# DavidSlayback/po-brax

Hardware: AMD Instinct MI355X
Metric: env-steps/sec AntHeavenHell batch 65536 @1/2/4/8 GPU; % HBM roofline (higher is better)
Workload: dtype f32; 1 GPU; ant_heavenhell B=65536/GPU (global 65536), create(batch_size=B) autoreset chain, episode_length 1000, PBD 10 substeps, random uniform(-1,1) actions (threefry); env=ant_heavenhell, global_batch=65536, batch_per_gpu=65536, episode_length=1000, qp_storage=f32, parallelism=env-shard x1 (strong: global batch split), dynamics=pbd, obs_mask=none, obs_mask_columns=0, launch=hipGraph replay of the K steps

## Files before the change

__graft_entry__.py:

```python
from __future__ import annotations

import os
import subprocess
import sys
import sysconfig

ROOT = os.path.dirname(os.path.abspath(__file__))
PKG_ROOT = os.path.join(ROOT, "po-brax_amd")
CSRC = os.path.join(PKG_ROOT, "csrc")
LIB = os.path.join(PKG_ROOT, "po_brax_amd", "libpob.so")
HIP_SOURCES = ["pob_kernels.hip", "pob_system.cpp"]
HIP_DEPS = HIP_SOURCES + ["pob_math.h", "pob_mesh.h", "pob_physics.h", "pob_quad.h", "pob_octet.h", "pob_hexa.h", "pob_sys.h"]
HIPCC_FLAGS = ["--offload-arch=gfx950", "-O3", "-std=c++17", "-ffp-contract=off", "-fno-fast-math",
               "-fno-slp-vectorize", "-fPIC", "-shared", "-mcode-object-version=5", "-Wall",
               "-Wno-unused-result"]

if PKG_ROOT not in sys.path:
    sys.path.insert(0, PKG_ROOT)


def _stale(target, deps):
    if not os.path.exists(target):
        return True
    t = os.path.getmtime(target)
    return any(os.path.getmtime(d) > t for d in deps)


def build_lib(force: bool = False) -> str:
    deps = [os.path.join(CSRC, f) for f in HIP_DEPS] + [os.path.join(ROOT, "include", "pob.h")]
    if force or _stale(LIB, deps):
        hipcc = os.environ.get("HIPCC", "/opt/rocm/bin/hipcc")
        cmd = [hipcc, *HIPCC_FLAGS, "-o", LIB, *[os.path.join(CSRC, f) for f in HIP_SOURCES]]
        subprocess.check_call(cmd)
    return LIB

# ... 61 lines not shown
```

po-brax_amd/csrc/pob_kernels.hip:

```cpp
#include <hip/hip_fp16.h>
#include <hip/hip_runtime.h>

#include <climits>
#include <cstdio>
#include <cstdlib>
#include <cstring>
#include <mutex>
#include <new>
#include <type_traits>
#include <vector>

#include "../../include/pob.h"

#ifndef POB_QUAD_PRIO
#define POB_QUAD_PRIO 1
#endif
#ifndef POB_OCT_PRIO
#define POB_OCT_PRIO 1
#endif
#ifndef POB_HEX_PRIO
#define POB_HEX_PRIO 1
#endif
#include "pob_quad.h"
#include "pob_octet.h"
#include "pob_hexa.h"
#include "pob_physics.h"

namespace pob {
void default_params(pob_params &p);
const char *build_system(int kind, const pob_params &p, pob_sys &s);
int gather_grid(const pob_params &p, float *xyz, int cap);
}

struct pob_env {
  pob_sys sys;
  pob_sys *d_sys = nullptr;
  pob_params params;
  float *d_grid = nullptr;
  uint32_t *d_scratch = nullptr;
  int device = 0;
  int n_cu = 256;
};

#define POB_MIXED (-1)
#define POB_F_STAGED (1u << 16)
#define POB_F_INT_FORCE_FIXUP (1u << 30)
#define POB_F_INTERNAL (POB_F_STAGED | POB_F_INT_FORCE_FIXUP)
#define POB_F_PUBLIC (POB_F_EPISODE | POB_F_AUTORESET | POB_F_ZERO_STEPS_ON_DONE)

#define POB_STATE_FIELDS(X)                                                                    \
  X(pos) X(rot) X(vel) X(ang) X(obs) X(reward) X(done) X(steps) X(truncation) X(m0) X(m1) X(m2) \
  X(rng) X(first_pos) X(first_rot) X(first_vel) X(first_ang) X(first_obs) X(any_done) X(done_u8) X(trunc_i32) \
  X(m0_i32) X(m1_i32) X(any_done_clear) X(obs_masked) X(ovf_mark)

struct StatePtrs {
  float *pos, *rot, *vel, *ang, *obs, *reward, *done, *steps, *truncation, *m0, *m1, *m2;
  uint32_t *rng;
  float *first_pos, *first_rot, *first_vel, *first_ang, *first_obs;
  uint32_t *any_done;
  uint8_t *done_u8;
  int32_t *trunc_i32, *m0_i32, *m1_i32;
  uint32_t *any_done_clear;
  float *obs_masked;
  uint8_t *ovf_mark;
};
POB_D void store_obs_masked(csys_t &S, float *dst, const float *stg, const int rows, const int D, const int lane) {
  const int K = S.obs_mask_n;
  for (int r = 0; r < rows; ++r)
    for (int c = lane; c < K; c += 64) dst[(size_t)r * K + c] = stg[r * D + S.obs_mask[c]];
}
// ... 555 lines not shown
#pragma unroll
      for (int l = 0; l < QNB; ++l) {
        if (l == 0 && k != 0) continue;
        const int g = qbody_global(l, k);
        float *o = stg + (le * POB_NDYN + g) * c;
        if (reset_rows) {
          const float *F = arr == 0 ? in.first_pos : (arr == 1 ? in.first_rot : (arr == 2 ? in.first_vel : in.first_ang));
          const size_t src = (arr == 1 ? r4 : r3) + (size_t)g * c;
          for (int q = 0; q < c; ++q) o[q] = Q<QT>::ld(F, src + q);
        } else if (arr == 0) { o[0] = bd.x[l].x; o[1] = bd.x[l].y; o[2] = bd.x[l].z; }
        else if (arr == 1) { o[0] = bd.q[l].w; o[1] = bd.q[l].x; o[2] = bd.q[l].y; o[3] = bd.q[l].z; }
        else if (arr == 2) { o[0] = bd.v[l].x; o[1] = bd.v[l].y; o[2] = bd.v[l].z; }
        else { o[0] = bd.w[l].x; o[1] = bd.w[l].y; o[2] = bd.w[l].z; }
      }
    }
    wave_lds_sync();
    if (arr == 1) stage_store_dyn<QT, 4>(out.rot, (size_t)b_first * N * 4, N, nenv, stg, lane);
    else stage_store_dyn<QT, 3>(arr == 0 ? out.pos : (arr == 2 ? out.vel : out.ang), (size_t)b_first * N * 3, N,
                                nenv, stg, lane);
    wave_lds_sync();
  }
}

template <int KIND, typename QT, bool LEG = false, int MODE = 0>
POB_D void step_quad_body(csys_t *Sp, const int B, const StatePtrs &in, const float *__restrict__ act,
                          const StatePtrs &out, const uint32_t flags, const int L, const int gt, float *lds,
                          const float *legtab) {
  csys_t &S = *Sp;
  const int lane = (int)threadIdx.x & 63;
  POB_TS_DECL();
  POB_TS(0);
  float *stg = lds + ((int)threadIdx.x >> 6) * POB_STAGE_FLOATS;
  const QLds Ls{stg, lane};
  int b = gt >> 2;
  int k = gt & 3;
  const float *LT = legtab + k * POB_LEG_FLOATS;
  const float *WT = legtab + 4 * POB_LEG_FLOATS;
  const int kind = KIND != POB_MIXED ? KIND : S.kind;
  const int N = n_bodies<KIND>(S), D = obs_dim<KIND>(S);
  const int sh = obs_shift(kind);
  bool act_lane = b < B;
  int b_first = (gt - lane) >> 2;
  if (b_first >= B) return;
  if (MODE == 2 && out.ovf_mark[b_first] == 0) return;
  if (MODE == 1 && lane == 0) out.ovf_mark[b_first] = 0;
  int nenv = B - b_first < 16 ? B - b_first : 16;
  int le = b - b_first;
  int bl = act_lane ? b : B - 1, lel = bl - b_first;
  size_t r3 = (size_t)bl * N * 3, r4 = (size_t)bl * N * 4;
  auto rederive = [&]() {
    int g2 = gt;
    asm volatile("" : "+v"(g2));
    b = g2 >> 2;
    k = g2 & 3;
    act_lane = b < B;
    b_first = (g2 - (g2 & 63)) >> 2;
    nenv = B - b_first < 16 ? B - b_first : 16;
    le = b - b_first;
    bl = act_lane ? b : B - 1;
    lel = bl - b_first;
    r3 = (size_t)bl * N * 3;
    r4 = (size_t)bl * N * 4;
  };

  QBody bd;
  constexpr int NMAX = KIND == POB_HEAVENHELL ? 14 : (KIND == POB_TAG ? 12 : (KIND == POB_ANT ? 10 : POB_MAXB));
  constexpr int MAXI = (16 * NMAX * 4 + 255) / 256;
  if ((flags & POB_F_STAGED) && NMAX <= 16 && N == NMAX && 16 * N * 7 <= POB_STAGE_FLOATS) {
// ... 110 lines not shown
    };
    for (;;) {
    if (pass == 0) {
      bool near = false;
#pragma nounroll
      for (int it = 0; it < 2 * iters; ++it) {
#if POB_QUAD_PRIO == 1
        const int lvl = (it * 4) / (2 * iters);
        if (lvl == 0) __builtin_amdgcn_s_setprio(3);
        else if (lvl == 1) __builtin_amdgcn_s_setprio(2);
        else if (lvl == 2) __builtin_amdgcn_s_setprio(1);
        else __builtin_amdgcn_s_setprio(0);
#endif
        qpbd_substep<false, true>(Sp, LT, WT, bd, a, Ls, (it & 1) != 0, fric, &near);
      }
      if (!__any(near)) break;
      pass = 1;
      reload();
      continue;
    }
#ifndef POB_QUAD_SLOW_OOL
#define POB_QUAD_SLOW_OOL 1
#endif
    if (MODE == 1 && WALLS) {
      bool ovf = false;
#pragma nounroll
      for (int it = 0; it < 2 * iters; ++it) {
#if POB_QUAD_PRIO == 1
        const int lvl = (it * 4) / (2 * iters);
        if (lvl == 0) __builtin_amdgcn_s_setprio(3);
        else if (lvl == 1) __builtin_amdgcn_s_setprio(2);
        else if (lvl == 2) __builtin_amdgcn_s_setprio(1);
        else __builtin_amdgcn_s_setprio(0);
#endif
        qpbd_substep<WALLS, false, false>(Sp, LT, WT, bd, a, Ls, (it & 1) != 0, fric, nullptr, &ovf);
        if (__any(ovf)) break;
      }
      if (__any(ovf) || (flags & POB_F_INT_FORCE_FIXUP)) {
        if (lane == 0) out.ovf_mark[b_first] = 1;
        return;
      }
      break;
    }
    if (pass == 1 && WALLS && FASTP && MODE == 0) {
      bool ovf = false;
#pragma nounroll
// ... 188 lines not shown
    if (out.truncation) out.truncation[b] = t.trunc;
    if (out.m0) out.m0[b] = t.m0;
    if (out.m1) out.m1[b] = t.m1;
    if (out.m2) out.m2[b] = t.m2;
    out.rng[2 * b] = t.rng0;
    out.rng[2 * b + 1] = t.rng1;
    write_typed(out, b, t);
  }
  if (out.any_done) {
    const unsigned long long m = __ballot(act_lane && k == 0 && done != 0.0f);
    if (m != 0ull && lane == 0) atomicOr(out.any_done, 1u);
  }
  POB_TS_WRITE();
}

POB_D bool quad_block_marked(const int B, const uint8_t *mark, const int bt0) {
  bool any = false;
  for (int w = 0; w < (int)blockDim.x / 64; ++w) {
    const int bf = (bt0 + 64 * w) >> 2;
    if (bf < B) any = any | (mark[bf] != 0);
  }
  return any;
}
template <int KIND, typename QT, int MODE = 0>
__global__ __launch_bounds__(256, POB_QUAD_MIN_WAVES) void k_step_quad(const void *sysp, const int B,
                                                                       const StatePtrs in,
                                                                       const float *__restrict__ act,
                                                                       const StatePtrs out, const uint32_t flags,
                                                                       const int L) {
  __shared__ float lds[QL_FLOATS * 256];
  __shared__ __attribute__((aligned(16))) float legtab[POB_TAB_FLOATS];
  if (MODE == 2 && !quad_block_marked(B, out.ovf_mark, (int)(blockIdx.x * blockDim.x)))
    return;
  stage_leg_table((csys_t *)(size_t)sysp, legtab);
  step_quad_body<KIND, QT, false, MODE>((csys_t *)(size_t)sysp, B, in, act, out, flags, L,
                                        (int)(blockIdx.x * blockDim.x + threadIdx.x), lds, legtab);
}

template <typename QT>
__global__ __launch_bounds__(256, 3) void k_step_quad_ga3(const void *sysp, const int B, const StatePtrs in,
                                                          const float *__restrict__ act, const StatePtrs out,
                                                          const uint32_t flags, const int L) {
  __shared__ float lds[QL_FLOATS * 256];
  __shared__ __attribute__((aligned(16))) float legtab[POB_TAB_FLOATS];
  stage_leg_table((csys_t *)(size_t)sysp, legtab);
  step_quad_body<POB_GATHER, QT>((csys_t *)(size_t)sysp, B, in, act, out, flags, L,
                                 (int)(blockIdx.x * blockDim.x + threadIdx.x), lds, legtab);
}

template <int KIND, typename QT>
__global__ __launch_bounds__(256) void k_step_legacy(const void *sysp, const int B, const StatePtrs in,
                                                     const float *__restrict__ act, const StatePtrs out,
                                                     const uint32_t flags, const int L) {
  __shared__ float lds[QL_FLOATS * 256];
  __shared__ __attribute__((aligned(16))) float legtab[POB_TAB_FLOATS];
  stage_leg_table((csys_t *)(size_t)sysp, legtab);
  step_quad_body<KIND, QT, true>((csys_t *)(size_t)sysp, B, in, act, out, flags, L,
                                 (int)(blockIdx.x * blockDim.x + threadIdx.x), lds, legtab);
// ... 1420 lines not shown
    default: hipLaunchKernelGGL((k_step_oct<POB_ANT, QT, GACC>), g, b, 0, st, sp, B, pi, act, po, flags, L); break;
  }
}
template <typename QT>
static void launch_step_oct(int kind, int n_cu, hipStream_t st, const void *sp, int B, const StatePtrs &pi,
                            const float *act, const StatePtrs &po, uint32_t flags, int L) {
  const char *f = getenv("POB_OCT_GACC");
  const bool acc = f ? atoi(f) != 0 : (B + 7) / 8 <= 4 * n_cu;
  if (acc) launch_step_oct_g<QT, true>(kind, st, sp, B, pi, act, po, flags, L);
  else launch_step_oct_g<QT, false>(kind, st, sp, B, pi, act, po, flags, L);
}
#ifndef POB_QUAD_SPLIT_KINDS
#define POB_QUAD_SPLIT_KINDS 23
#endif
static bool quad_split_launch(int kind) {
  const char *f = getenv("POB_QUAD_SPLIT");
  if (f) return atoi(f) != 0;
  return ((POB_QUAD_SPLIT_KINDS >> (kind < 0 ? 4 : kind)) & 1) != 0;
}
static uint32_t quad_force_fixup() {
  const char *f = getenv("POB_QUAD_FORCE_FIXUP");
  return f && atoi(f) != 0 ? POB_F_INT_FORCE_FIXUP : 0u;
}
template <typename QT>
static void launch_step_quad(int kind, bool legacy, int n_cu, hipStream_t st, const void *sp, int B,
                             const StatePtrs &pi, const float *act, const StatePtrs &po, uint32_t flags, int L) {
  const int bs = 4 * B <= 64 * 256 ? 64 : 256;
  const dim3 g = grid_for(4 * B, bs), b(bs);
  if (legacy) {
    switch (kind) {
      case POB_HEAVENHELL: hipLaunchKernelGGL((k_step_legacy<POB_HEAVENHELL, QT>), g, b, 0, st, sp, B, pi, act, po, flags, L); break;
      case POB_GATHER: hipLaunchKernelGGL((k_step_legacy<POB_GATHER, QT>), g, b, 0, st, sp, B, pi, act, po, flags, L); break;
      case POB_TAG: hipLaunchKernelGGL((k_step_legacy<POB_TAG, QT>), g, b, 0, st, sp, B, pi, act, po, flags, L); break;
      default: hipLaunchKernelGGL((k_step_legacy<POB_ANT, QT>), g, b, 0, st, sp, B, pi, act, po, flags, L); break;
    }
    return;
  }
  if (kind == POB_GATHER && (size_t)4 * B <= (size_t)3 * 64 * 4 * n_cu) {
    hipLaunchKernelGGL((k_step_quad_ga3<QT>), g, b, 0, st, sp, B, pi, act, po, flags, L);
    return;
  }
  const bool split = quad_split_launch(kind) && po.ovf_mark != nullptr;
  flags |= split ? quad_force_fixup() : 0u;
  switch (kind) {
    case POB_HEAVENHELL:
      if (split) {
        hipLaunchKernelGGL((k_step_quad<POB_HEAVENHELL, QT, 1>), g, b, 0, st, sp, B, pi, act, po, flags, L);
        hipLaunchKernelGGL((k_step_quad<POB_HEAVENHELL, QT, 2>), g, b, 0, st, sp, B, pi, act, po, flags, L);
      } else {
        hipLaunchKernelGGL((k_step_quad<POB_HEAVENHELL, QT>), g, b, 0, st, sp, B, pi, act, po, flags, L);
      }
      break;
    case POB_GATHER:
      if (split) {
        hipLaunchKernelGGL((k_step_quad<POB_GATHER, QT, 1>), g, b, 0, st, sp, B, pi, act, po, flags, L);
        hipLaunchKernelGGL((k_step_quad<POB_GATHER, QT, 2>), g, b, 0, st, sp, B, pi, act, po, flags, L);
      } else {
        hipLaunchKernelGGL((k_step_quad<POB_GATHER, QT>), g, b, 0, st, sp, B, pi, act, po, flags, L);
      }
      break;
    case POB_TAG:
      if (split) {
        hipLaunchKernelGGL((k_step_quad<POB_TAG, QT, 1>), g, b, 0, st, sp, B, pi, act, po, flags, L);
        hipLaunchKernelGGL((k_step_quad<POB_TAG, QT, 2>), g, b, 0, st, sp, B, pi, act, po, flags, L);
      } else {
        hipLaunchKernelGGL((k_step_quad<POB_TAG, QT>), g, b, 0, st, sp, B, pi, act, po, flags, L);
      }
      break;
    default: hipLaunchKernelGGL((k_step_quad<POB_ANT, QT>), g, b, 0, st, sp, B, pi, act, po, flags, L); break;
  }
}
extern "C" {

int pob_abi_version(void) { return POB_ABI_VERSION; }
const char *pob_last_error(void) { return g_err; }

int pob_default_params(pob_params *p) {
  if (!p) return fail(POB_EINVAL, "params is NULL");
  pob::default_params(*p);
  return POB_OK;
}

static std::mutex g_grave_mu;
static std::vector<void *> g_grave;

static void drain_grave() {
// ... 303 lines not shown
```

po-brax_amd/csrc/pob_mesh.h:

```cpp
#pragma once
#include <type_traits>
#include "pob_math.h"

#define POB_MESH_MARGIN 1e-3f
#if defined(POB_MESH_HOST) || defined(POB_FC_LDS)
typedef const float *fcptr_t;
#else
typedef __attribute__((address_space(4))) const float *fcptr_t;
#endif

struct MWall {
  float cx, cy, c, s, hx, hy;
};
POB_D MWall mwall_row(const float *R) {
  const float2 r01 = *reinterpret_cast<const float2 *>(R);
  const float2 r23 = *reinterpret_cast<const float2 *>(R + 2);
  const float2 r45 = *reinterpret_cast<const float2 *>(R + 4);
  MWall W;
  W.cx = r01.x; W.cy = r01.y; W.c = r23.x; W.s = r23.y; W.hx = r45.x; W.hy = r45.y;
  return W;
}
POB_D v3 mwall_local(const MWall &W, const float cz, const v3 p) {
  const float dx = p.x - W.cx, dy = p.y - W.cy, dz = p.z - cz;
  return V(FMA(dy, W.s, dx * W.c), FMA(dy, W.c, -(dx * W.s)), dz);
// ... 437 lines not shown
#define POB_MESH_NOINLINE 0
#endif
template <class G, class Fn>
POB_D void mesh_face(G &g, const int f, const v3 La, const v3 Lb, const float hx, const float hy, const float hz,
                     fcptr_t fcw, const float r, const float T, Fn &&emit) {
#if POB_MESH_NOINLINE && !defined(POB_MESH_HOST)
  if constexpr (std::is_same<G, GuardBranch>::value) {
    const MFaceOut o = mesh_face_ool(f, La, Lb, hx, hy, hz, fcw, r, T);
    if (o.hit[0]) emit(o.tau[0], o.nl[0], o.dist[0]);
    if (o.hit[1]) emit(o.tau[1], o.nl[1], o.dist[1]);
    return;
  }
#endif
  const MFaceOut o = mesh_face_contacts(g, f, La, Lb, hx, hy, hz, fcw, r, T);
  if (o.hit[0]) emit(o.tau[0], o.nl[0], o.dist[0]);
  if (o.hit[1]) emit(o.tau[1], o.nl[1], o.dist[1]);
}

POB_D v3 mwall_world_n(const MWall &W, const v3 nl) {
  return V(FMA(-nl.y, W.s, nl.x * W.c), FMA(nl.y, W.c, nl.x * W.s), nl.z);
}

#ifndef POB_MESH_HOST
static_assert(POB_MAXW <= 8, "face items pack wall w and face f as bit 8 w + f of a uint64_t");
POB_D float mlane_read(const float v, const int src) {
  return __int_as_float(__builtin_amdgcn_ds_bpermute(src << 2, __float_as_int(v)));
}
POB_D int mlane_read_i(const int v, const int src) { return __builtin_amdgcn_ds_bpermute(src << 2, v); }
template <int CTRL>
POB_D void mlexmin_dpp(float &d, int &kk) {
  const float od = __int_as_float(__builtin_amdgcn_mov_dpp(__float_as_int(d), CTRL, 0xf, 0xf, true));
  const int ok = __builtin_amdgcn_mov_dpp(kk, CTRL, 0xf, 0xf, true);
  const bool take = (od < d) | ((od == d) & (ok < kk));
  d = take ? od : d;
  kk = take ? ok : kk;
}
template <int CTRL>
POB_D int msum_dpp(const int v) { return v + __builtin_amdgcn_mov_dpp(v, CTRL, 0xf, 0xf, true); }
template <int J>
POB_D float mquad_read(const float v) {
  return __int_as_float(__builtin_amdgcn_mov_dpp(__float_as_int(v), J * 0x55, 0xf, 0xf, true));
}
template <int J>
POB_D void mtie_add(const float key, const float dmin, const F3 S, const F3 P, const float u, F3 &Ss, F3 &Ps,
                    float &us, float &cnt) {
  const float kj = mquad_read<J>(key);
// ... 188 lines not shown
    if constexpr (HAND == 2) {
      const int e = apply.store(hit, tau, nw, dst);
      const int eq = msum_dpp<0x4E>(msum_dpp<0xB1>(e));
      const int e10 = mlane_read_i(eq, g1), e11 = mlane_read_i(eq, g1 + 4);
      const int e20 = mlane_read_i(eq, g2), e21 = mlane_read_i(eq, g2 + 4);
      if (own1) { apply.link(s, b1, e10); apply.link(s, b1, e11); }
      if (own2) { apply.link(s, b2, e20); apply.link(s, b2, e21); }
    } else {
      const int w10 = g1 + mlane_read_i(kmin, g1), w11 = g1 + 4 + mlane_read_i(kmin, g1 + 4);
      const int w20 = g2 + mlane_read_i(kmin, g2), w21 = g2 + 4 + mlane_read_i(kmin, g2 + 4);
      const int nt = __any(own2) ? 4 : 2;
#pragma nounroll
      for (int t = 0; t < nt; ++t) {
        const int wl = t == 0 ? w10 : (t == 1 ? w11 : (t == 2 ? w20 : w21));
        const int h = mlane_read_i(hit ? 1 : 0, wl);
        const float tw = mlane_read(tau, wl), dw = mlane_read(dst, wl);
        const v3 nn = V(mlane_read(nw.x, wl), mlane_read(nw.y, wl), mlane_read(nw.z, wl));
        if constexpr (HAND == 1) apply((t < 2 ? own1 : own2) && h != 0, s, t < 2 ? b1 : b2, tw, nn, dw);
        else if ((t < 2 ? own1 : own2) && h != 0) apply(s, t < 2 ? b1 : b2, tw, nn, dw);
      }
    }
  }
}
#endif
```

po-brax_amd/csrc/pob_quad.h:

```cpp
#pragma once
#include "pob_physics.h"

#define QNB 3
#define QNJ 2

struct QBody {
  v3 x[QNB];
  q4 q[QNB];
  v3 v[QNB];
  v3 w[QNB];
};

template <int J>
POB_D float quad_bcast(float x) {
  float r;
  if (J == 0)
    asm volatile("s_nop 1\n\tv_mov_b32_dpp %0, %1 quad_perm:[0,0,0,0] row_mask:0xf bank_mask:0xf" : "=&v"(r) : "v"(x));
  else if (J == 1)
    asm volatile("s_nop 1\n\tv_mov_b32_dpp %0, %1 quad_perm:[1,1,1,1] row_mask:0xf bank_mask:0xf" : "=&v"(r) : "v"(x));
  else if (J == 2)
    asm volatile("s_nop 1\n\tv_mov_b32_dpp %0, %1 quad_perm:[2,2,2,2] row_mask:0xf bank_mask:0xf" : "=&v"(r) : "v"(x));
  else
    asm volatile("s_nop 1\n\tv_mov_b32_dpp %0, %1 quad_perm:[3,3,3,3] row_mask:0xf bank_mask:0xf" : "=&v"(r) : "v"(x));
  return r;
// ... 77 lines not shown
  return V(e[0], e[1], e[2]);
}
POB_D v3 qground_end(csys_t &S, const float *LT, int c) {
  if (c == 0) return SV(S.ground_end[0]);
  return V(LT[POB_LEG_GROUND], LT[POB_LEG_GROUND + 1], LT[POB_LEG_GROUND + 2]);
}
POB_D float qground_r(csys_t &S, const float *LT, int c) {
  return c == 0 ? S.ground_r[0] : LT[POB_LEG_GROUND + 3];
}

struct QGround {
  float pen[2];
};
struct QMesh {
  v3 a[QNB], b[QNB];
};
#ifndef QK
#define QK 12
#endif
struct QWalls {
  int nct;
  float c[6 * QK];
  float seg[6 * QNB];
};
#ifndef POB_QUAD_WAVE_WALK
#define POB_QUAD_WAVE_WALK 1
#endif
#if POB_QUAD_WAVE_WALK
#define QWALK mesh_wave_walk
#else
#define QWALK mesh_lane_walk
#endif

POB_D void qground_detect(csys_t &S, const float *LT, const QBody &b, const v3 rv_leg, QGround &gc, v3 (&pe)[2]) {
  pe[0] = S.torso_point ? b.x[0] : vadd(b.x[0], qrot(qground_end(S, LT, 0), b.q[0]));
  pe[1] = vsub(b.x[2], rv_leg);
  gc.pen[0] = qground_r(S, LT, 0) - pe[0].z;
  gc.pen[1] = qground_r(S, LT, 1) - pe[1].z;
}

POB_D uint32_t qwall_mask(csys_t &S, const QBody &b) {
  float mnx = b.x[0].x, mxx = b.x[0].x, mny = b.x[0].y, mxy = b.x[0].y;
#pragma unroll
  for (int l = 1; l < QNB; ++l) {
    mnx = fminf(mnx, b.x[l].x); mxx = fmaxf(mxx, b.x[l].x);
    mny = fminf(mny, b.x[l].y); mxy = fmaxf(mxy, b.x[l].y);
// ... 155 lines not shown
        else *head = __int_as_float(idx);
        tail = idx;
        tail_l = l;
      }
    }
  }
};
#ifndef POB_QUAD_WALK_GACC
#define POB_QUAD_WALK_GACC 0
#endif
POB_D void qwalls_walk_pool(csys_t &S, const float *LT, const float *WT, const QBody &b, uint64_t (&M)[QNB],
                            QWalls &ws, const QLds &L, bool &ovf) {
#if POB_QUAD_WALK_GACC
  GuardAcc g;
#else
  GuardBranch g;
#endif
#if POB_QUAD_POOL_DIRECT
  QPoolSink sink{L.pool(), L.head(), 0, -1, 0, 0};
  mesh_wave_walk<QNB, false, 2>(g, WT, pob_face_table(S), S.wall_cz, S.wall_hz, M,
             [&](const int l, v3 &A, v3 &B, float &r, bool &seg) { qpose_seg(S, LT, b, l, A, B, r, seg); }, sink);
  ws.nct += sink.nct;
  ovf = ovf | (sink.npool > QPOOL_N);
#if POB_QUAD_WALK_GACC
  ovf = ovf | g.bad();
#endif
  return;
#endif
  float *pool = L.pool();
  int npool = 0;
  int tail = -1, tail_l = 0;
  mesh_wave_walk<QNB, false, 1>(g, WT, pob_face_table(S), S.wall_cz, S.wall_hz, M,
             [&](const int l, v3 &A, v3 &B, float &r, bool &seg) { qpose_seg(S, LT, b, l, A, B, r, seg); },
             [&](const bool want, const int l, const int, const float tau, const v3 n, const float dist) {
    const uint64_t m = __ballot(want);
    if (m == 0ull) return;
    const int idx = npool + (int)__builtin_amdgcn_mbcnt_hi((uint32_t)(m >> 32), __builtin_amdgcn_mbcnt_lo((uint32_t)m, 0u));
    npool += __popcll(m);
    if (want) {
      if (idx < QPOOL_N) {
        float *c = pool + 6 * idx;
        c[0] = tau; c[1] = n.x; c[2] = n.y; c[3] = n.z; c[4] = dist; c[5] = __int_as_float(l);
        if (tail >= 0) pool[6 * tail + 5] = __int_as_float(((idx + 1) << 2) | tail_l);
        else *L.head() = __int_as_float(idx);
        tail = idx;
        tail_l = l;
// ... 46 lines not shown
#endif
#ifdef POB_EXP_NO_APPLY
  {
    int z = ws.nct & 0;
    asm volatile("" : "+v"(z));
    ws.nct = z;
  }
#endif
  if (!OVF) {
    *ovf = *ovf | (ws.nct > QK);
    return;
  }
  if (ws.nct > QK) {
    QMesh ms;
    qmesh_segments(S, LT, b, rv_leg, ms);
#pragma unroll
    for (int l = 0; l < QNB; ++l) {
      ws.seg[6 * l] = ms.a[l].x; ws.seg[6 * l + 1] = ms.a[l].y; ws.seg[6 * l + 2] = ms.a[l].z;
      ws.seg[6 * l + 3] = ms.b[l].x; ws.seg[6 * l + 4] = ms.b[l].y; ws.seg[6 * l + 5] = ms.b[l].z;
    }
  }
}

template <class G>
POB_D void qwall_pos_one(G &g, csys_t &S, const HCon &SC, const float *LT, const v3 (&x)[QNB], const q4 (&q)[QNB],
                         const v3 (&px)[QNB], const q4 (&pq)[QNB], const int l, const float tau, const v3 n,
                         const float dist, v3 (&DX)[QNB], v3 (&DA)[QNB]) {
  const v3 xl = qpick3(l, x);
  const q4 ql = qpick4(l, q);
  const v3 pe = l == 0 ? xl : qseg_point(LT, l, xl, ql, tau);
  v3 dx = qpick3(l, DX), da = qpick3(l, DA);
  owall_position(g, SC, q_cap_r(S, LT, l) - dist, pe, n, 1e-6f + dist, q_inv_mass(S, LT, l), xl, ql, qpick4(l, pq),
                 qpick3(l, px), dx, da);
  qput3(l, DX, dx);
  qput3(l, DA, da);
}
template <class G>
POB_D void qwall_vel_one(G &g, csys_t &S, const HCon &SC, const float *LT, const v3 (&x)[QNB], const q4 (&q)[QNB],
                         const v3 (&v)[QNB], const v3 (&w)[QNB], const int l, const float tau, const v3 n,
                         const float dist, v3 (&dV)[QNB], v3 (&dW)[QNB]) {
  const v3 xl = qpick3(l, x);
  const v3 pe = l == 0 ? xl : qseg_point(LT, l, xl, qpick4(l, q), tau);
  v3 dv = qpick3(l, dV), dw = qpick3(l, dW);
  ocontact_vel_pe(g, SC, false, q_cap_r(S, LT, l) - dist, pe, n, 1e-6f + dist, q_inv_mass(S, LT, l), xl, qpick3(l, v),
                  qpick3(l, w), dv, dw);
  qput3(l, dV, dv);
// ... 44 lines not shown
#pragma unroll
  for (int l = 0; l < QNB; ++l) {
    ms.a[l] = V(ws.seg[6 * l], ws.seg[6 * l + 1], ws.seg[6 * l + 2]);
    ms.b[l] = V(ws.seg[6 * l + 3], ws.seg[6 * l + 4], ws.seg[6 * l + 5]);
  }
  const uint32_t wa = ovf ? (1u << S.n_walls) - 1u : 0u;
  uint64_t M[QNB];
  qmesh_items(S, LT, WT, wa | (wa << 8) | (wa << 16), ms, M);
  mesh_wave_walk<QNB, false>(g, WT, pob_face_table(S), S.wall_cz, S.wall_hz, M,
             [&](const int l, v3 &A, v3 &B, float &r, bool &seg) { qmesh_seg(S, LT, ms, l, A, B, r, seg); },
             [&](const int l, const int, const float tau, const v3 n, const float dist) {
    if constexpr (VEL) {
      qwall_vel_one(g, S, SC, LT, b.x, b.q, b.v, b.w, l, tau, n, dist, d0, d1);
    } else {
      v3 px[QNB];
      q4 pq[QNB];
#pragma unroll
      for (int k = 0; k < QNB; ++k) { px[k] = L.get3(k, QF_PX); pq[k] = L.get4(k, QF_PQ); }
      qwall_pos_one(g, S, SC, LT, b.x, b.q, px, pq, l, tau, n, dist, d0, d1);
    }
  });
}

template <bool WALLS, bool OVF = true>
POB_D void qcontacts_position(csys_t *Sp, const float *LT, const float *WT, QBody &b, const QLds &L, QGround &gc,
                              const QWalls &ws, v3 (&DX)[QNB], v3 (&DA)[QNB], const float fric) {
  csys_t &S = *launder(Sp);
  const HCon SC{fric, S.inv_h};
  GuardBranch g;
  {
    const v3 rv_leg = qrot_xy(qcap_end(S, LT, 2, 0), b.q[2]);
    v3 pe[2];
    qground_detect(S, LT, b, rv_leg, gc, pe);
#pragma unroll
    for (int c = 0; c < 2; ++c) {
      POB_FENCE();
      const int l = qcontact_body(c);
      if (gc.pen[c] > 0.0f)
        oground_position(g, SC, gc.pen[c], pe[c], qground_r(S, LT, c), q_inv_mass(S, LT, l), b.x[l], b.q[l],
                         L.get4(l, QF_PQ), L.get3(l, QF_PX), DX[l], DA[l]);
    }
  }
  if (!WALLS || !__any(ws.nct != 0)) return;
  POB_FENCE();
  v3 px[QNB];
  q4 pq[QNB];
#pragma unroll
  for (int l = 0; l < QNB; ++l) { px[l] = L.get3(l, QF_PX); pq[l] = L.get4(l, QF_PQ); }
#if POB_QUAD_WAVE_WALK
  if (!OVF) {
    const float *pool = L.pool();
    int ci = ws.nct > 0 ? __float_as_int(*L.head()) : -1;
#pragma unroll 1
    while (__any(ci >= 0)) {
      if (ci >= 0) {
        const float *c = pool + 6 * ci;
        const int meta = __float_as_int(c[5]);
        qwall_pos_one(g, S, SC, LT, b.x, b.q, px, pq, meta & 3, c[0], V(c[1], c[2], c[3]), c[4], DX, DA);
        ci = (meta >> 2) - 1;
      }
    }
    return;
  }
#endif
  const bool ovf = ws.nct > QK;
  const int nc = ovf ? 0 : ws.nct;
#pragma unroll 1
  for (int i = 0; i < QK; ++i) {
    if (!__any(i < nc)) break;
    if (i < nc) {
      const float *c = ws.c + 6 * i;
// ... 4 lines not shown
#if POB_QUAD_REWALK_INLINE
#ifndef POB_EXP_NO_REWALK
  if (__any(ovf)) qwalls_rewalk_inl<false>(S, LT, WT, b, L, ws, ovf, fric, DX, DA);
#endif
  if (false) {
#else
  if (__any(ovf)) {
#endif
    QOvf st;
#pragma unroll
    for (int l = 0; l < QNB; ++l) {
      st.x[l] = b.x[l]; st.q[l] = b.q[l]; st.px[l] = px[l]; st.pq[l] = pq[l]; st.d0[l] = DX[l]; st.d1[l] = DA[l];
      st.a[l] = V(ws.seg[6 * l], ws.seg[6 * l + 1], ws.seg[6 * l + 2]);
      st.b[l] = V(ws.seg[6 * l + 3], ws.seg[6 * l + 4], ws.seg[6 * l + 5]);
    }
    st.fric = fric;
    st.on = ovf ? 1 : 0;
    qwalls_rewalk<false>(Sp, LT, WT, &st);
#pragma unroll
    for (int l = 0; l < QNB; ++l) { DX[l] = st.d0[l]; DA[l] = st.d1[l]; b.x[l] = st.x[l]; b.q[l] = st.q[l]; }
  }
}

template <bool WALLS, bool OVF = true>
POB_D void qcontacts_velocity(csys_t *Sp, const float *LT, const float *WT, QBody &b, const QGround &gc,
                              const QWalls &ws, const QLds &L, v3 (&dV)[QNB], v3 (&dW)[QNB], const float fric) {
  csys_t &S = *launder(Sp);
  const HCon SC{fric, S.inv_h};
  GuardBranch g;
#pragma unroll
  for (int c = 0; c < 2; ++c) {
    POB_FENCE();
    const int l = qcontact_body(c);
    if (gc.pen[c] > 0.0f) {
      const v3 e = qground_end(S, LT, c);
      const v3 pe = l == 0 ? vadd(b.x[0], qrot(e, b.q[0])) : vadd(b.x[l], qrot_xy(e, b.q[l]));
      ocontact_vel_pe(g, SC, true, gc.pen[c], pe, V(0.0f, 0.0f, 1.0f), qground_r(S, LT, c), q_inv_mass(S, LT, l), b.x[l],
                      b.v[l], b.w[l], dV[l], dW[l]);
    }
  }
  if (!WALLS || !__any(ws.nct != 0)) return;
#ifdef POB_EXP_NO_VWALK
  return;
#endif
  POB_FENCE();
#if POB_QUAD_WAVE_WALK
  if (!OVF) {
    const float *pool = L.pool();
    int ci = ws.nct > 0 ? __float_as_int(*L.head()) : -1;
#pragma unroll 1
    while (__any(ci >= 0)) {
      if (ci >= 0) {
        const float *c = pool + 6 * ci;
        const int meta = __float_as_int(c[5]);
        qwall_vel_one(g, S, SC, LT, b.x, b.q, b.v, b.w, meta & 3, c[0], V(c[1], c[2], c[3]), c[4], dV, dW);
        ci = (meta >> 2) - 1;
      }
    }
    return;
  }
#endif
  const bool ovf = ws.nct > QK;
  const int nc = ovf ? 0 : ws.nct;
#pragma unroll 1
  for (int i = 0; i < QK; ++i) {
    if (!__any(i < nc)) break;
    if (i < nc) {
      const float *c = ws.c + 6 * i;
// ... 130 lines not shown
  const v3 tp = vadd(xp, s);
  if (torso_parent) tt->t = tp;
  else DA[p] = vadd(DA[p], tp);
  DA[c] = vsub(DA[c], vadd(xc, s));
}

template <int J>
POB_D void qtorso_add(v3 &dx, v3 &da, const QTorso &t, const float imp0) {
  dx = vfma(quad_bcast3<J>(t.P), imp0, dx);
  da = vadd(da, quad_bcast3<J>(t.t));
}

#ifndef POB_QFRIC_REG
#define POB_QFRIC_REG 1
#endif
POB_D float quad_friction(const csys_t &S) {
  float f = S.friction;
#if POB_QFRIC_REG
  asm volatile("" : "+s"(f));
#endif
  return f;
}

template <bool WALLS, bool CHECK = false, bool OVF = true>
POB_D void qpbd_substep(csys_t *Sp, const float *LT, const float *WT, QBody &b, const float (&act)[QNJ], const QLds &L,
                        const bool COLLIDE, const float fric, bool *near = nullptr, bool *ovf = nullptr) {
#pragma unroll
  for (int l = 0; l < QNB; ++l) { L.set3(l, QF_PX, b.x[l]); L.set4(l, QF_PQ, b.q[l]); }
  {
    v3 tt[QNJ];
#pragma unroll
    for (int jl = 0; jl < QNJ; ++jl) {
      const int p = jparent(jl), c = jchild(jl);
      const v3 axis = QJV(LT, jl, QJ_AXIS);
      const v3 a = jl == 0 ? qrot_ez(b.q[p]) : qrot_xy(axis, b.q[p]);
      const bool in = actuator_inside(b.q[p], b.q[c], jl == 0, axis, QJS(LT, jl, QJ_TLO), QJS(LT, jl, QJ_THI));
      v3 t = vscl(a, (in ? act[jl] : 0.0f) * QJS(LT, jl, QJ_STRENGTH));
      v3 d = vscl(vsub(b.w[p], b.w[c]), QJS(LT, jl, QJ_DAMP));
      tt[jl] = vadd(t, d);
    }
    v3 dw[QNB];
    {
      const v3 t0 = quad_bcast3<0>(tt[0]), t2 = quad_bcast3<1>(tt[0]);
      const v3 t4 = quad_bcast3<2>(tt[0]), t6 = quad_bcast3<3>(tt[0]);
      dw[0] = vsub(vsub(vsub(vsub(V(0.0f, 0.0f, 0.0f), t0), t2), t4), t6);
    }
    dw[1] = vsub(vadd(V(0.0f, 0.0f, 0.0f), tt[0]), tt[1]);
    dw[2] = vadd(V(0.0f, 0.0f, 0.0f), tt[1]);
    csys_t &S = *launder(Sp);
#pragma unroll
    for (int l = 0; l < QNB; ++l) {
      const v3 v = b.v[l], w = b.w[l];
      b.v[l] = V(FMA(S.lin_damp, v.x, 0.0f * S.h), FMA(S.lin_damp, v.y, 0.0f * S.h), FMA(S.lin_damp, v.z, S.gz * S.h));
      b.w[l] = V(FMA(S.ang_damp, w.x, dw[l].x * S.h), FMA(S.ang_damp, w.y, dw[l].y * S.h),
                 FMA(S.ang_damp, w.z, dw[l].z * S.h));
    }
#pragma unroll
    for (int l = 0; l < QNB; ++l) {
      b.x[l] = vfma(b.v[l], S.h, b.x[l]);
      q4 dq = qmul_vq(b.w[l], b.q[l]);
      q4 q = b.q[l];
      q.w = FMA(S.half_h, dq.w, q.w); q.x = FMA(S.half_h, dq.x, q.x);
      q.y = FMA(S.half_h, dq.y, q.y); q.z = FMA(S.half_h, dq.z, q.z);
      b.q[l] = qnormalize(q);
    }
  }
  QWalls ws;
  ws.nct = 0;
  if (COLLIDE) qwalls_detect<WALLS, OVF>(Sp, LT, WT, b, ws, L, ovf);
  if (CHECK && COLLIDE) *near = *near | (qwall_mask(*launder(Sp), b) != 0u);
  QGround gc;
  {
    v3 DX[QNB];
    v3 DA[QNB];
#pragma unroll
    for (int l = 0; l < QNB; ++l) { DX[l] = V(0.0f, 0.0f, 0.0f); DA[l] = V(0.0f, 0.0f, 0.0f); }
    QTorso tq;
    POB_FENCE();
#ifdef POB_EXP_NO_JOINTS
    tq.P = V(0.0f, 0.0f, 0.0f);
    tq.t = tq.P;
#else
    qjoint_position(Sp, LT, b, 0, DX, DA, &tq);
#ifndef POB_EXP_JOINT_ILP
    POB_FENCE();
#endif
    qjoint_position(Sp, LT, b, 1, DX, DA, nullptr);
#endif
    POB_FENCE();
    {
      const float imp0 = launder(Sp)->inv_mass[0];
      qtorso_add<0>(DX[0], DA[0], tq, imp0);
      qtorso_add<1>(DX[0], DA[0], tq, imp0);
      qtorso_add<2>(DX[0], DA[0], tq, imp0);
      qtorso_add<3>(DX[0], DA[0], tq, imp0);
    }
    if (COLLIDE) qcontacts_position<WALLS, OVF>(Sp, LT, WT, b, L, gc, ws, DX, DA, fric);
#pragma unroll
    for (int l = 0; l < QNB; ++l) {
      b.x[l] = vadd(b.x[l], DX[l]);
      qadd_half(b.q[l], qmul_vq(DA[l], b.q[l]), 1.0f);
    }
  }
#pragma unroll
  for (int l = 0; l < QNB; ++l) {
    csys_t &S = *launder(Sp);
    b.q[l] = qnormalize(b.q[l]);
    b.v[l] = vscl(vsub(b.x[l], L.get3(l, QF_PX)), S.inv_h);
    q4 dq = qmul(b.q[l], qinv(L.get4(l, QF_PQ)));
    const float k2 = 2.0f * S.inv_h;
    const float kw = dq.w >= 0.0f ? k2 : -k2;
    b.w[l] = V(dq.x * kw, dq.y * kw, dq.z * kw);
  }
  if (COLLIDE) {
    v3 dV[QNB], dW[QNB];
#pragma unroll
    for (int l = 0; l < QNB; ++l) { dV[l] = V(0.0f, 0.0f, 0.0f); dW[l] = V(0.0f, 0.0f, 0.0f); }
    qcontacts_velocity<WALLS, OVF>(Sp, LT, WT, b, gc, ws, L, dV, dW, fric);
#pragma unroll
    for (int l = 0; l < QNB; ++l) {
      b.v[l] = vadd(b.v[l], dV[l]); b.w[l] = vadd(b.w[l], dW[l]);
      L.set3(l, QF_CV, vadd(L.get3(l, QF_CV), dV[l]));
      L.set3(l, QF_CA, vadd(L.get3(l, QF_CA), dW[l]));
    }
  }
}

struct QSlow {
  QBody b;
  float act[QNJ];
};
template <bool WALLS>
__device__ __attribute__((noinline)) void qpbd_substep_slow(csys_t *Sp, const float *LT, const float *WT, QSlow *st,
                                                           float *lbase, const int lt, const int collide,
                                                           const float fric) {
  QBody b = st->b;
  float act[QNJ];
#pragma unroll
  for (int j = 0; j < QNJ; ++j) act[j] = st->act[j];
  const QLds L{lbase, lt};
  qpbd_substep<WALLS>(Sp, LT, WT, b, act, L, collide != 0, fric);
// ... 85 lines not shown
```

Measured before the change: 459.7 million env-steps/s.

## Add block-cooperative wall contact walk sharing items across four waves

```diff
diff --git a/__graft_entry__.py b/__graft_entry__.py
--- a/__graft_entry__.py
+++ b/__graft_entry__.py
@@ -10,7 +10,7 @@
 CSRC = os.path.join(PKG_ROOT, "csrc")
 LIB = os.path.join(PKG_ROOT, "po_brax_amd", "libpob.so")
 HIP_SOURCES = ["pob_kernels.hip", "pob_system.cpp"]
-HIP_DEPS = HIP_SOURCES + ["pob_math.h", "pob_mesh.h", "pob_physics.h", "pob_quad.h", "pob_octet.h", "pob_hexa.h", "pob_sys.h"]
+HIP_DEPS = HIP_SOURCES + ["pob_math.h", "pob_mesh.h", "pob_blockwalk.h", "pob_physics.h", "pob_quad.h", "pob_octet.h", "pob_hexa.h", "pob_sys.h"]
 HIPCC_FLAGS = ["--offload-arch=gfx950", "-O3", "-std=c++17", "-ffp-contract=off", "-fno-fast-math",
                "-fno-slp-vectorize", "-fPIC", "-shared", "-mcode-object-version=5", "-Wall",
                "-Wno-unused-result"]
diff --git a/po-brax_amd/csrc/pob_blockwalk.h b/po-brax_amd/csrc/pob_blockwalk.h
--- /dev/null
+++ b/po-brax_amd/csrc/pob_blockwalk.h
@@ -0,0 +1,73 @@
+#pragma once
+#include <stdint.h>
+#ifdef POB_BW_HOST
+#define POB_BW_D static inline
+#else
+#define POB_BW_D __device__ __forceinline__
+#endif
+
+#define QBW_WAVES 4
+#define QBW_WCAP 50
+#define QBW_SLOT_DW 11
+#define QBW_CON_DW 5
+#define QBW_LANE_MAX 64
+#define QBW_CAP (QBW_WAVES * QBW_WCAP)
+#define QBW_SEG_FLOATS (QBW_WCAP * QBW_SLOT_DW + 1)
+#define QBW_NO_CONTACT (-1)
+
+POB_BW_D constexpr int bw_item_off(const int j) { return QBW_SLOT_DW * j; }
+POB_BW_D constexpr int bw_meta_off(const int j) { return QBW_SLOT_DW * j + 2 * QBW_CON_DW; }
+POB_BW_D constexpr int bw_con_off(const int c) { return QBW_SLOT_DW * (c >> 1) + QBW_CON_DW * (c & 1); }
+POB_BW_D constexpr int bw_count_off() { return QBW_WCAP * QBW_SLOT_DW; }
+
+POB_BW_D constexpr int bw_meta(const int bit, const bool seg, const int slot) { return bit | (seg ? 64 : 0) | (slot << 7); }
+POB_BW_D constexpr int bw_meta_bit(const int m) { return m & 63; }
+POB_BW_D constexpr bool bw_meta_seg(const int m) { return (m & 64) != 0; }
+POB_BW_D constexpr int bw_meta_slot(const int m) { return (m >> 7) & 3; }
+
+POB_BW_D int bw_lane_count(const uint64_t m0, const uint64_t m1, const uint64_t m2) {
+  const int n = __builtin_popcountll(m0) + __builtin_popcountll(m1) + __builtin_popcountll(m2);
+  return n < QBW_LANE_MAX ? n : QBW_LANE_MAX;
+}
+POB_BW_D void bw_prefix_step(const uint64_t m, const int lane, const int b, int &base, int &tot) {
+  base += __builtin_popcountll(m & ((1ull << lane) - 1ull)) << b;
+  tot += __builtin_popcountll(m) << b;
+}
+#define QBW_PREFIX_BITS 7
+
+POB_BW_D bool bw_next_item(uint64_t (&M)[3], int &slot, int &bit) {
+  const bool h0 = M[0] != 0ull, h1 = M[1] != 0ull, h2 = M[2] != 0ull;
+  const bool has = h0 | h1 | h2;
+  slot = h0 ? 0 : (h1 ? 1 : 2);
+  const uint64_t ml = h0 ? M[0] : (h1 ? M[1] : M[2]);
+  bit = has ? __builtin_ctzll(ml) : 0;
+  const uint64_t pop = has ? ml & (0ull - ml) : 0ull;
+  M[0] = h0 ? M[0] & ~pop : M[0];
+  M[1] = (!h0 & h1) ? M[1] & ~pop : M[1];
+  M[2] = (!h0 & !h1) ? M[2] & ~pop : M[2];
+  return has;
+}
+
+struct BwDeal {
+  int off[QBW_WAVES];
+  int T;
+  bool ovf;
+};
+POB_BW_D BwDeal bw_deal(const int n0, const int n1, const int n2, const int n3, const int cap) {
+  BwDeal d;
+  d.off[0] = 0; d.off[1] = n0; d.off[2] = n0 + n1; d.off[3] = n0 + n1 + n2;
+  const int T = n0 + n1 + n2 + n3;
+  d.ovf = (T > cap) | (n0 > QBW_WCAP) | (n1 > QBW_WCAP) | (n2 > QBW_WCAP) | (n3 > QBW_WCAP);
+  d.T = d.ovf ? 0 : T;
+  return d;
+}
+POB_BW_D int bw_rounds(const BwDeal &d) { return (d.T + 7) >> 3; }
+POB_BW_D int bw_first_round(const int w, const int sub) { return (w + sub) & (QBW_WAVES - 1); }
+POB_BW_D void bw_item_owner(const BwDeal &d, const int i, int &w, int &j) {
+  w = (i >= d.off[1] ? 1 : 0) + (i >= d.off[2] ? 1 : 0) + (i >= d.off[3] ? 1 : 0);
+  j = i - (w == 0 ? 0 : (w == 1 ? d.off[1] : (w == 2 ? d.off[2] : d.off[3])));
+}
+POB_BW_D void bw_apply_range(const int base, const int n, const bool ovf, int &c0, int &c1) {
+  c0 = 2 * base;
+  c1 = ovf ? c0 : 2 * (base + n);
+}
diff --git a/po-brax_amd/csrc/pob_kernels.hip b/po-brax_amd/csrc/pob_kernels.hip
--- a/po-brax_amd/csrc/pob_kernels.hip
+++ b/po-brax_amd/csrc/pob_kernels.hip
@@ -45,7 +45,9 @@
 #define POB_MIXED (-1)
 #define POB_F_STAGED (1u << 16)
 #define POB_F_INT_FORCE_FIXUP (1u << 30)
-#define POB_F_INTERNAL (POB_F_STAGED | POB_F_INT_FORCE_FIXUP)
+#define POB_F_INT_BWCAP_SHIFT 20
+#define POB_F_INT_BWCAP_MASK (0xFFu << POB_F_INT_BWCAP_SHIFT)
+#define POB_F_INTERNAL (POB_F_STAGED | POB_F_INT_FORCE_FIXUP | POB_F_INT_BWCAP_MASK)
 #define POB_F_PUBLIC (POB_F_EPISODE | POB_F_AUTORESET | POB_F_ZERO_STEPS_ON_DONE)
 
 #define POB_STATE_FIELDS(X)                                                                    \
@@ -647,7 +649,7 @@
   }
 }
 
-template <int KIND, typename QT, bool LEG = false, int MODE = 0>
+template <int KIND, typename QT, bool LEG = false, int MODE = 0, bool COOP = false>
 POB_D void step_quad_body(csys_t *Sp, const int B, const StatePtrs &in, const float *__restrict__ act,
                           const StatePtrs &out, const uint32_t flags, const int L, const int gt, float *lds,
                           const float *legtab) {
@@ -666,9 +668,11 @@
   const int sh = obs_shift(kind);
   bool act_lane = b < B;
   int b_first = (gt - lane) >> 2;
-  if (b_first >= B) return;
+  const bool dead = b_first >= B;
+  if (!COOP && dead) return;
   if (MODE == 2 && out.ovf_mark[b_first] == 0) return;
-  if (MODE == 1 && lane == 0) out.ovf_mark[b_first] = 0;
+  if (MODE == 1 && lane == 0 && !dead) out.ovf_mark[b_first] = 0;
+  if (COOP && dead) b_first = ((B - 1) >> 4) << 4;
   int nenv = B - b_first < 16 ? B - b_first : 16;
   int le = b - b_first;
   int bl = act_lane ? b : B - 1, lel = bl - b_first;
@@ -825,6 +829,28 @@
 #ifndef POB_QUAD_SLOW_OOL
 #define POB_QUAD_SLOW_OOL 1
 #endif
+    if constexpr (MODE == 1 && WALLS && COOP) {
+      const int capf = (int)((flags & POB_F_INT_BWCAP_MASK) >> POB_F_INT_BWCAP_SHIFT);
+      QBlock blk{lds + QPOOL_OFF, __builtin_amdgcn_readfirstlane((int)threadIdx.x >> 6), 0,
+                 capf != 0 ? capf : QBW_CAP, dead, false};
+#pragma nounroll
+      for (int it = 0; it < 2 * iters; ++it) {
+#if POB_QUAD_PRIO == 1
+        const int lvl = (it * 4) / (2 * iters);
+        if (lvl == 0) __builtin_amdgcn_s_setprio(3);
+        else if (lvl == 1) __builtin_amdgcn_s_setprio(2);
+        else if (lvl == 2) __builtin_amdgcn_s_setprio(1);
+        else __builtin_amdgcn_s_setprio(0);
+#endif
+        qpbd_substep<WALLS, false, false, true>(Sp, LT, WT, bd, a, Ls, (it & 1) != 0, fric, nullptr, nullptr, &blk);
+      }
+      if (dead) return;
+      if (blk.ovf || (flags & POB_F_INT_FORCE_FIXUP)) {
+        if (lane == 0) out.ovf_mark[b_first] = 1;
+        return;
+      }
+      break;
+    }
     if (MODE == 1 && WALLS) {
       bool ovf = false;
 #pragma nounroll
@@ -1059,18 +1085,19 @@
   }
   return any;
 }
-template <int KIND, typename QT, int MODE = 0>
+template <int KIND, typename QT, int MODE = 0, bool COOP = false>
 __global__ __launch_bounds__(256, POB_QUAD_MIN_WAVES) void k_step_quad(const void *sysp, const int B,
                                                                        const StatePtrs in,
                                                                        const float *__restrict__ act,
                                                                        const StatePtrs out, const uint32_t flags,
                                                                        const int L) {
-  __shared__ float lds[QL_FLOATS * 256];
+  static_assert(!COOP || (MODE == 1 && (KIND == POB_HEAVENHELL || KIND == POB_TAG)), "the cooperative walk: fast launch, HH / TAG");
+  __shared__ __attribute__((aligned(16))) float lds[QL_FLOATS * 256];
   __shared__ __attribute__((aligned(16))) float legtab[POB_TAB_FLOATS];
   if (MODE == 2 && !quad_block_marked(B, out.ovf_mark, (int)(blockIdx.x * blockDim.x)))
     return;
   stage_leg_table((csys_t *)(size_t)sysp, legtab);
-  step_quad_body<KIND, QT, false, MODE>((csys_t *)(size_t)sysp, B, in, act, out, flags, L,
+  step_quad_body<KIND, QT, false, MODE, COOP>((csys_t *)(size_t)sysp, B, in, act, out, flags, L,
                                         (int)(blockIdx.x * blockDim.x + threadIdx.x), lds, legtab);
 }
 
@@ -2537,6 +2564,11 @@
   const char *f = getenv("POB_QUAD_FORCE_FIXUP");
   return f && atoi(f) != 0 ? POB_F_INT_FORCE_FIXUP : 0u;
 }
+static uint32_t quad_block_cap() {
+  const char *f = getenv("POB_QUAD_BLOCK_CAP");
+  const int n = f ? atoi(f) : 0;
+  return n >= 1 && n < QBW_CAP ? (uint32_t)n << POB_F_INT_BWCAP_SHIFT : 0u;
+}
 template <typename QT>
 static void launch_step_quad(int kind, bool legacy, int n_cu, hipStream_t st, const void *sp, int B,
                              const StatePtrs &pi, const float *act, const StatePtrs &po, uint32_t flags, int L) {
@@ -2557,10 +2589,13 @@
   }
   const bool split = quad_split_launch(kind) && po.ovf_mark != nullptr;
   flags |= split ? quad_force_fixup() : 0u;
+  const bool coop = split && bs == 256 && (kind == POB_HEAVENHELL || kind == POB_TAG);
+  flags |= coop ? quad_block_cap() : 0u;
   switch (kind) {
     case POB_HEAVENHELL:
       if (split) {
-        hipLaunchKernelGGL((k_step_quad<POB_HEAVENHELL, QT, 1>), g, b, 0, st, sp, B, pi, act, po, flags, L);
+        if (coop) hipLaunchKernelGGL((k_step_quad<POB_HEAVENHELL, QT, 1, true>), g, b, 0, st, sp, B, pi, act, po, flags, L);
+        else hipLaunchKernelGGL((k_step_quad<POB_HEAVENHELL, QT, 1>), g, b, 0, st, sp, B, pi, act, po, flags, L);
         hipLaunchKernelGGL((k_step_quad<POB_HEAVENHELL, QT, 2>), g, b, 0, st, sp, B, pi, act, po, flags, L);
       } else {
         hipLaunchKernelGGL((k_step_quad<POB_HEAVENHELL, QT>), g, b, 0, st, sp, B, pi, act, po, flags, L);
@@ -2576,7 +2611,8 @@
       break;
     case POB_TAG:
       if (split) {
-        hipLaunchKernelGGL((k_step_quad<POB_TAG, QT, 1>), g, b, 0, st, sp, B, pi, act, po, flags, L);
+        if (coop) hipLaunchKernelGGL((k_step_quad<POB_TAG, QT, 1, true>), g, b, 0, st, sp, B, pi, act, po, flags, L);
+        else hipLaunchKernelGGL((k_step_quad<POB_TAG, QT, 1>), g, b, 0, st, sp, B, pi, act, po, flags, L);
         hipLaunchKernelGGL((k_step_quad<POB_TAG, QT, 2>), g, b, 0, st, sp, B, pi, act, po, flags, L);
       } else {
         hipLaunchKernelGGL((k_step_quad<POB_TAG, QT>), g, b, 0, st, sp, B, pi, act, po, flags, L);
diff --git a/po-brax_amd/csrc/pob_mesh.h b/po-brax_amd/csrc/pob_mesh.h
--- a/po-brax_amd/csrc/pob_mesh.h
+++ b/po-brax_amd/csrc/pob_mesh.h
@@ -483,6 +483,7 @@
 }
 
 #ifndef POB_MESH_HOST
+#include "pob_blockwalk.h"
 static_assert(POB_MAXW <= 8, "face items pack wall w and face f as bit 8 w + f of a uint64_t");
 POB_D float mlane_read(const float v, const int src) {
   return __int_as_float(__builtin_amdgcn_ds_bpermute(src << 2, __float_as_int(v)));
@@ -717,4 +718,58 @@
     }
   }
 }
-#endif
+
+template <class G>
+POB_D void mesh_block_walk(G &g, const float *WT, fcptr_t FC, const float cz, const float hz, float *xch,
+                           const int wstride, const BwDeal &d, const int r0) {
+  const int lane = (int)__lane_id();
+  const int grp = lane >> 3, tri = (lane >> 2) & 1, kk = lane & 3;
+  const int R = bw_rounds(d);
+#pragma nounroll
+  for (int r = r0; r < R; r += QBW_WAVES) {
+    const int i = 8 * r + grp;
+    const bool gv = i < d.T;
+    int ow, j;
+    bw_item_owner(d, gv ? i : 0, ow, j);
+    float *sg = xch + ow * wstride;
+    const float *rec = sg + bw_item_off(j);
+    const v3 Ao = V(rec[0], rec[1], rec[2]), Bo = V(rec[3], rec[4], rec[5]);
+    const float ro = rec[6];
+    const int mo = __float_as_int(rec[7]);
+    const bool sego = bw_meta_seg(mo);
+    const MWall W = mwall_row(WT + POB_WALL_FLOATS * ((mo >> 3) & 7));
+    fcptr_t fcw = FC + 3 * POB_FACE_FLOATS * ((mo >> 3) & 7);
+    const v3 La = mwall_local(W, cz, Ao);
+    const v3 Lb = sego ? mwall_local(W, cz, Bo) : La;
+    const MFace F = mface(g, mo & 7, mcap_seg(g, La, Lb), W.hx, W.hy, hz, fcw);
+    F3 Sc, Pc;
+    MCand c = mface_cand_quad(g, F, tri, gv ? kk : 7, Sc, Pc);
+    c.d2 = mcand_key(c.d2);
+    float dmin = c.d2;
+    int kmin = kk;
+    mlexmin_dpp<0xB1>(dmin, kmin);
+    mlexmin_dpp<0x4E>(dmin, kmin);
+    const int neq = msum_dpp<0x4E>(msum_dpp<0xB1>(c.d2 == dmin ? 1 : 0));
+    const float T = (ro * ro) * 1.00000095367431640625f;
+    const bool tie = gv && neq > 1 && dmin < T;
+    if (__any(tie)) {
+      F3 Ss = f3(0.0f, 0.0f, 0.0f), Ps = Ss;
+      float us = 0.0f, cnt = 0.0f;
+      mtie_add<0>(c.d2, dmin, Sc, Pc, c.u, Ss, Ps, us, cnt);
+      mtie_add<1>(c.d2, dmin, Sc, Pc, c.u, Ss, Ps, us, cnt);
+      mtie_add<2>(c.d2, dmin, Sc, Pc, c.u, Ss, Ps, us, cnt);
+      mtie_add<3>(c.d2, dmin, Sc, Pc, c.u, Ss, Ps, us, cnt);
+      if (tie && kk == kmin) c = bcand(f3(Ss.a / cnt, Ss.b / cnt, Ss.w / cnt), f3(Ps.a / cnt, Ps.b / cnt, Ps.w / cnt), us / cnt);
+    }
+    if (gv && kk == kmin) {
+      float tau = 0.0f, dst = 0.0f;
+      v3 nl, nw = V(0.0f, 0.0f, 0.0f);
+      const bool hit = mface_contact(g, F.k, c, ro, T, tau, nl, dst);
+      if (hit) nw = mwall_world_n(W, nl);
+      float *o = sg + bw_con_off(2 * j + tri);
+      o[0] = tau; o[1] = nw.x; o[2] = nw.y; o[3] = nw.z;
+      o[4] = hit ? dst : __int_as_float(QBW_NO_CONTACT);
+    }
+  }
+}
+#endif
diff --git a/po-brax_amd/csrc/pob_quad.h b/po-brax_amd/csrc/pob_quad.h
--- a/po-brax_amd/csrc/pob_quad.h
+++ b/po-brax_amd/csrc/pob_quad.h
@@ -123,6 +123,7 @@
   int nct;
   float c[6 * QK];
   float seg[6 * QNB];
+  int c0, c1;
 };
 #ifndef POB_QUAD_WAVE_WALK
 #define POB_QUAD_WAVE_WALK 1
@@ -324,6 +325,7 @@
              [&](const int l, v3 &A, v3 &B, float &r, bool &seg) { qpose_seg(S, LT, b, l, A, B, r, seg); }, sink);
   ws.nct += sink.nct;
   ovf = ovf | (sink.npool > QPOOL_N);
+  if (sink.npool > QPOOL_N) ws.nct = 0;
 #if POB_QUAD_WALK_GACC
   ovf = ovf | g.bad();
 #endif
@@ -416,6 +418,83 @@
   }
 }
 
+struct QBlock {
+  float *xch;
+  int w;
+  int sub;
+  int cap;
+  bool dead;
+  bool ovf;
+};
+static_assert(QBW_SEG_FLOATS <= QL_FLOATS * 64 - QPOOL_OFF, "a wave's exchange segment fits its former contact pool");
+POB_D void qblock_barrier() { asm volatile("s_waitcnt lgkmcnt(0)\n\ts_barrier" ::: "memory"); }
+
+POB_D void qwalls_detect_block(csys_t *Sp, const float *LT, const float *WT, const QBody &b, QWalls &ws, const QLds &L,
+                               QBlock &blk) {
+  csys_t &S = *launder(Sp);
+  uint64_t M[QNB];
+  {
+    const v3 rv_leg = qrot_xy(qcap_end(S, LT, 2, 0), b.q[2]);
+    QMesh ms;
+    qmesh_segments(S, LT, b, rv_leg, ms);
+    const uint32_t lw = qwall_mask(S, b);
+    qmesh_items(S, LT, WT, lw | (lw << 8) | (lw << 16), ms, M);
+  }
+  if (blk.dead) { M[0] = 0ull; M[1] = 0ull; M[2] = 0ull; }
+  float *own = L.pool();
+  const int nl = bw_lane_count(M[0], M[1], M[2]);
+  int base = 0, tot = 0;
+#pragma unroll
+  for (int bit = 0; bit < QBW_PREFIX_BITS; ++bit) bw_prefix_step(__ballot(((nl >> bit) & 1) != 0), L.t, bit, base, tot);
+  {
+    int at = base;
+#pragma nounroll
+    for (int k = 0; k < QBW_LANE_MAX; ++k) {
+      int s, bit;
+      const bool has = bw_next_item(M, s, bit);
+      if (!__any(has)) break;
+      v3 A, B;
+      float r;
+      bool seg;
+      qpose_seg(S, LT, b, s, A, B, r, seg);
+      if (has && at < QBW_WCAP) {
+        float *o = own + bw_item_off(at);
+        const float meta = __int_as_float(bw_meta(bit, seg, s));
+        o[0] = A.x; o[1] = A.y; o[2] = A.z; o[3] = B.x; o[4] = B.y; o[5] = B.z; o[6] = r; o[7] = meta;
+        o[2 * QBW_CON_DW] = meta;
+      }
+      ++at;
+    }
+  }
+  if (L.t == 0) own[bw_count_off()] = __int_as_float(tot);
+  qblock_barrier();
+  const int ws_f = QL_FLOATS * 64;
+  const int n0 = __builtin_amdgcn_readfirstlane(__float_as_int(blk.xch[bw_count_off()]));
+  const int n1 = __builtin_amdgcn_readfirstlane(__float_as_int(blk.xch[ws_f + bw_count_off()]));
+  const int n2 = __builtin_amdgcn_readfirstlane(__float_as_int(blk.xch[2 * ws_f + bw_count_off()]));
+  const int n3 = __builtin_amdgcn_readfirstlane(__float_as_int(blk.xch[3 * ws_f + bw_count_off()]));
+  const BwDeal d = bw_deal(n0, n1, n2, n3, blk.cap);
+  blk.ovf = blk.ovf | d.ovf;
+  {
+    GuardBranch g;
+    mesh_block_walk(g, WT, pob_face_table(S), S.wall_cz, S.wall_hz, blk.xch, ws_f, d, bw_first_round(blk.w, blk.sub));
+  }
+  qblock_barrier();
+  ++blk.sub;
+  bw_apply_range(base, nl, d.ovf, ws.c0, ws.c1);
+  ws.nct = ws.c1 - ws.c0;
+}
+
+POB_D int qblock_next_hit(const float *sg, int c, const int c1) {
+#pragma unroll 1
+  while (true) {
+    const bool skip = c < c1 && __float_as_int(sg[bw_con_off(c) + QBW_CON_DW - 1]) == QBW_NO_CONTACT;
+    if (!__any(skip)) break;
+    c = skip ? c + 1 : c;
+  }
+  return c;
+}
+
 template <class G>
 POB_D void qwall_pos_one(G &g, csys_t &S, const HCon &SC, const float *LT, const v3 (&x)[QNB], const q4 (&q)[QNB],
                          const v3 (&px)[QNB], const q4 (&pq)[QNB], const int l, const float tau, const v3 n,
@@ -506,7 +585,7 @@
   });
 }
 
-template <bool WALLS, bool OVF = true>
+template <bool WALLS, bool OVF = true, bool COOP = false>
 POB_D void qcontacts_position(csys_t *Sp, const float *LT, const float *WT, QBody &b, const QLds &L, QGround &gc,
                               const QWalls &ws, v3 (&DX)[QNB], v3 (&DA)[QNB], const float fric) {
   csys_t &S = *launder(Sp);
@@ -531,6 +610,21 @@
   q4 pq[QNB];
 #pragma unroll
   for (int l = 0; l < QNB; ++l) { px[l] = L.get3(l, QF_PX); pq[l] = L.get4(l, QF_PQ); }
+  if constexpr (COOP) {
+    const float *sg = L.pool();
+    int c = qblock_next_hit(sg, ws.c0, ws.c1);
+#pragma unroll 1
+    while (__any(c < ws.c1)) {
+      if (c < ws.c1) {
+        const float *p = sg + bw_con_off(c);
+        const int l = bw_meta_slot(__float_as_int(sg[bw_meta_off(c >> 1)]));
+        qwall_pos_one(g, S, SC, LT, b.x, b.q, px, pq, l, p[0], V(p[1], p[2], p[3]), p[4], DX, DA);
+        ++c;
+      }
+      c = qblock_next_hit(sg, c, ws.c1);
+    }
+    return;
+  }
 #if POB_QUAD_WAVE_WALK
   if (!OVF) {
     const float *pool = L.pool();
@@ -581,7 +675,7 @@
   }
 }
 
-template <bool WALLS, bool OVF = true>
+template <bool WALLS, bool OVF = true, bool COOP = false>
 POB_D void qcontacts_velocity(csys_t *Sp, const float *LT, const float *WT, QBody &b, const QGround &gc,
                               const QWalls &ws, const QLds &L, v3 (&dV)[QNB], v3 (&dW)[QNB], const float fric) {
   csys_t &S = *launder(Sp);
@@ -603,6 +697,21 @@
   return;
 #endif
   POB_FENCE();
+  if constexpr (COOP) {
+    const float *sg = L.pool();
+    int c = qblock_next_hit(sg, ws.c0, ws.c1);
+#pragma unroll 1
+    while (__any(c < ws.c1)) {
+      if (c < ws.c1) {
+        const float *p = sg + bw_con_off(c);
+        const int l = bw_meta_slot(__float_as_int(sg[bw_meta_off(c >> 1)]));
+        qwall_vel_one(g, S, SC, LT, b.x, b.q, b.v, b.w, l, p[0], V(p[1], p[2], p[3]), p[4], dV, dW);
+        ++c;
+      }
+      c = qblock_next_hit(sg, c, ws.c1);
+    }
+    return;
+  }
 #if POB_QUAD_WAVE_WALK
   if (!OVF) {
     const float *pool = L.pool();
@@ -779,9 +888,10 @@
   return f;
 }
 
-template <bool WALLS, bool CHECK = false, bool OVF = true>
+template <bool WALLS, bool CHECK = false, bool OVF = true, bool COOP = false>
 POB_D void qpbd_substep(csys_t *Sp, const float *LT, const float *WT, QBody &b, const float (&act)[QNJ], const QLds &L,
-                        const bool COLLIDE, const float fric, bool *near = nullptr, bool *ovf = nullptr) {
+                        const bool COLLIDE, const float fric, bool *near = nullptr, bool *ovf = nullptr,
+                        QBlock *blk = nullptr) {
 #pragma unroll
   for (int l = 0; l < QNB; ++l) { L.set3(l, QF_PX, b.x[l]); L.set4(l, QF_PQ, b.q[l]); }
   {
@@ -824,7 +934,9 @@
   }
   QWalls ws;
   ws.nct = 0;
-  if (COLLIDE) qwalls_detect<WALLS, OVF>(Sp, LT, WT, b, ws, L, ovf);
+  if constexpr (COOP) {
+    if (COLLIDE) qwalls_detect_block(Sp, LT, WT, b, ws, L, *blk);
+  } else if (COLLIDE) qwalls_detect<WALLS, OVF>(Sp, LT, WT, b, ws, L, ovf);
   if (CHECK && COLLIDE) *near = *near | (qwall_mask(*launder(Sp), b) != 0u);
   QGround gc;
   {
@@ -852,7 +964,7 @@
       qtorso_add<2>(DX[0], DA[0], tq, imp0);
       qtorso_add<3>(DX[0], DA[0], tq, imp0);
     }
-    if (COLLIDE) qcontacts_position<WALLS, OVF>(Sp, LT, WT, b, L, gc, ws, DX, DA, fric);
+    if (COLLIDE) qcontacts_position<WALLS, OVF, COOP>(Sp, LT, WT, b, L, gc, ws, DX, DA, fric);
 #pragma unroll
     for (int l = 0; l < QNB; ++l) {
       b.x[l] = vadd(b.x[l], DX[l]);
@@ -873,7 +985,7 @@
     v3 dV[QNB], dW[QNB];
 #pragma unroll
     for (int l = 0; l < QNB; ++l) { dV[l] = V(0.0f, 0.0f, 0.0f); dW[l] = V(0.0f, 0.0f, 0.0f); }
-    qcontacts_velocity<WALLS, OVF>(Sp, LT, WT, b, gc, ws, L, dV, dW, fric);
+    qcontacts_velocity<WALLS, OVF, COOP>(Sp, LT, WT, b, gc, ws, L, dV, dW, fric);
 #pragma unroll
     for (int l = 0; l < QNB; ++l) {
       b.v[l] = vadd(b.v[l], dV[l]); b.w[l] = vadd(b.w[l], dW[l]);
```

Result: faster. 479.5 million env-steps/s (median of 6 runs) (+4.3%).
